# quadjr/aframe-gaussian-splatting

Measured on NVIDIA H100. Metric: frames/sec @1920x1080 (sort + splat raster, 1 M synthetic train-like splats), higher is better.
Workload: dtype f64 sort keys + f32 shading

## Files before the change

### aframe-gaussian-splatting_b200/csrc/gs_project.cu

```cuda
#include "gs_common.cuh"

namespace gs {

__device__ __forceinline__ void unpack_int16(uint32_t value, float &lo, float &hi) {
  const int32_t v = (int32_t)value;
  const int32_t v0 = v >> 16;
  int32_t v1 = v & 0xFFFF;
  if (v & 0x8000) v1 |= (int32_t)0xFFFF0000;
  lo = (float)v1;
  hi = (float)v0;
}

#define MUL(a, b) __fmul_rn((a), (b))
#define ADD(a, b) __fadd_rn((a), (b))
#define SUB(a, b) __fsub_rn((a), (b))
#define DIV(a, b) __fdiv_rn((a), (b))
#define DOT3(a0, b0, a1, b1, a2, b2) ADD(ADD(MUL(a0, b0), MUL(a1, b1)), MUL(a2, b2))

__device__ __forceinline__ uint32_t project_one(const RenderConsts &rc, const float *mv, const float4 c,
                                                const uint4 *__restrict__ cc, uint32_t i, uint32_t j,
                                                float4 *__restrict__ rec_out, uint4 &q, bool &have_q) {
  uint32_t rect = kNoRect;
  const float *P = rc.proj;
  float cam[4], p[4];
// ... 134 lines not shown
    constexpr uint32_t kChunk = 1024;
    __shared__ uint32_t s_list[kChunk];
    __shared__ uint32_t s_warp[8];
    const uint32_t tid = threadIdx.x, lane = tid & 31u, warp = tid >> 5;
    const uint32_t nchunks = (n + kChunk - 1) / kChunk;
    for (uint32_t ch = blockIdx.x; ch < nchunks; ch += gridDim.x) {
      const uint32_t base = ch * kChunk + tid * 4u;
      float d[4];
      if (base + 4u <= n) {
        const float4 v = __ldg((const float4 *)(depth + base));
        d[0] = v.x; d[1] = v.y; d[2] = v.z; d[3] = v.w;
        *(uint4 *)(rect_out + base) = make_uint4(kNoRect, kNoRect, kNoRect, kNoRect);
        if (STEREO) *(uint4 *)(rect_out1 + base) = make_uint4(kNoRect, kNoRect, kNoRect, kNoRect);
      } else {
#pragma unroll
        for (uint32_t k = 0; k < 4; ++k) {
          d[k] = (base + k < n) ? __ldg(depth + base + k) : GS_DEPTH_REJECT;
          if (base + k < n) rect_out[base + k] = kNoRect;
          if (STEREO && base + k < n) rect_out1[base + k] = kNoRect;
        }
      }
      bool f[4];
      uint32_t m = 0;
#pragma unroll
      for (uint32_t k = 0; k < 4; ++k) {
        f[k] = (base + k < n) && ((d[k] != GS_DEPTH_REJECT) || q5_head(base + k));
        m += f[k] ? 1u : 0u;
      }
      uint32_t incl = m;
      for (int o = 1; o < 32; o <<= 1) {
        const uint32_t t = __shfl_up_sync(0xffffffffu, incl, o);
        if (lane >= (uint32_t)o) incl += t;
      }
      if (lane == 31) s_warp[warp] = incl;
      __syncthreads();
      uint32_t pos = incl - m, total = 0;
#pragma unroll
      for (uint32_t w = 0; w < 8; ++w) {
        const uint32_t t = s_warp[w];
        pos += (w < warp) ? t : 0u;
        total += t;
      }
#pragma unroll
      for (uint32_t k = 0; k < 4; ++k)
        if (f[k]) s_list[pos++] = base + k;
      __syncthreads();
      for (uint32_t q = tid; q < total; q += blockDim.x) {
        const uint32_t i = s_list[q];
        uint32_t rect1 = kNoRect;
        const uint32_t rect = shade(i, i, &rect1);
        if (rect != kNoRect) rect_out[i] = rect;
        if (STEREO && rect1 != kNoRect) rect_out1[i] = rect1;
      }
      __syncthreads();
    }
    return;
  }
  for (uint32_t j = blockIdx.x * blockDim.x + threadIdx.x; j < n; j += stride) {
    const uint32_t i = BY_ENTRY ? __ldg(order + j) : j;
    uint32_t rect = kNoRect, rect1 = kNoRect;
    const bool sorted = BY_ENTRY || (__ldg(depth + i) != GS_DEPTH_REJECT) || q5_head(i);
    if (sorted) rect = shade(i, j, &rect1);
    rect_out[j] = rect;
    if (STEREO) rect_out1[j] = rect1;
  }
}


__device__ __forceinline__ uint32_t rect_count(uint32_t r, uint32_t rank, uint32_t world) {
  if (r == kNoRect) return 0u;
  const uint32_t h = (r >> 24) - ((r >> 16) & 255u) + 1u;
  uint32_t w = ((r >> 8) & 255u) - (r & 255u) + 1u;
  if (world > 1) {
    uint32_t first;
    owned_span(r & 255u, (r >> 8) & 255u, rank, world, first, w);
  }
  return w * h;
}

template <bool SLAB, bool STEREO = false>
__global__ void __launch_bounds__(kEmitThreads) k_count(const uint32_t *__restrict__ order,
                                                        const uint32_t *__restrict__ rect,
                                                        uint2 *__restrict__ ent, uint32_t *__restrict__ ent_off,
                                                        uint32_t *__restrict__ slice_total,
                                                        uint32_t *__restrict__ slice_prefix, FrameCounters *ctr,
                                                        const FrameParams *__restrict__ fp,
                                                        const uint32_t *__restrict__ bin_open,
                                                        uint32_t *__restrict__ rect1) {
  GS_PDL_ENTRY();
  const uint32_t shard_rank = fp->rc.shard_rank, shard_world = fp->rc.shard_world;
  __shared__ uint32_t s_warp[kEmitThreads / 32], s_vis[kEmitThreads / 32];
  __shared__ uint32_t s_last;
  const uint32_t tid = threadIdx.x, lane = tid & 31, warp = tid >> 5;
  const uint32_t nv = ctr->sort.n_valid;
  const uint32_t num_slices = (nv + kEmitTile - 1) / kEmitTile;
  for (uint32_t sl = blockIdx.x; sl < num_slices; sl += gridDim.x) {
    const uint32_t j = sl * kEmitTile + tid;
    uint32_t idx = 0, r = kNoRect, r1 = kNoRect;
    if (j < nv) {
      idx = SLAB ? j : __ldg(order + j);
      r = __ldg(rect + idx);
      if (STEREO) r1 = SLAB ? rect1[idx] : __ldg(rect1 + idx);
    }
    auto all_closed = [&](uint32_t rr, uint32_t bin_base) -> bool {
      const uint32_t bx0 = rr & 255u, bx1 = (rr >> 8) & 255u, by0 = (rr >> 16) & 255u, by1 = rr >> 24;
      if ((bx1 - bx0 + 1u) * (by1 - by0 + 1u) > 4u) return false;
      bool any = false;
      for (uint32_t by = by0; by <= by1; ++by)
        for (uint32_t bx = bx0; bx <= bx1; ++bx) any = any || (__ldg(bin_open + bin_base + by * fp->rc.bins_x + bx) != 0u);
      return !any;
    };
    uint32_t cnt = rect_count(r, shard_rank, shard_world);
    if (SLAB && cnt && all_closed(r, 0u)) cnt = 0;
    const uint32_t cnt0 = cnt;
    if (STEREO) {
      uint32_t cnt1 = rect_count(r1, 0u, 1u);
      if (SLAB && cnt1 && all_closed(r1, fp->rc.n_bins)) {
        cnt1 = 0;
        rect1[idx] = kNoRect;
      }
      cnt += cnt1;
    }
    uint32_t incl = cnt, vis = (r != kNoRect) + (STEREO && r1 != kNoRect);
    for (int o = 1; o < 32; o <<= 1) {
      const uint32_t t = __shfl_up_sync(0xffffffffu, incl, o);
      if (lane >= (uint32_t)o) incl += t;
    }
    for (int o = 16; o > 0; o >>= 1) vis += __shfl_xor_sync(0xffffffffu, vis, o);
    if (lane == 31) s_warp[warp] = incl;
    if (lane == 0) s_vis[warp] = vis;
    __syncthreads();
    uint32_t wbase = 0, total = 0, v = 0;
    for (uint32_t k = 0; k < kEmitThreads / 32; ++k) {
      if (k < warp) wbase += s_warp[k];
      total += s_warp[k];
      v += s_vis[k];
    }
    if (j < nv) {
      ent[j] = make_uint2(idx, (SLAB && STEREO ? cnt0 : cnt) ? r : kNoRect);
      ent_off[j] = wbase + incl - cnt;
    }
    if (tid == 0) {
      slice_total[sl] = total;
      if (v) atomicAdd(&ctr->n_visible, v);
    }
    __syncthreads();
  }
  __threadfence();
  __syncthreads();
  if (tid == 0) s_last = (atomicAdd(&ctr->count_done, 1u) == gridDim.x - 1) ? 1u : 0u;
  __syncthreads();
  if (!s_last) return;
  __threadfence();
  unsigned long long carry = 0;
  for (uint32_t b = 0; b < num_slices; b += kEmitThreads) {
    const uint32_t i = b + tid;
    const uint32_t v = (i < num_slices) ? __ldcg(slice_total + i) : 0u;
    uint32_t incl = v;
    for (int o = 1; o < 32; o <<= 1) {
      const uint32_t t = __shfl_up_sync(0xffffffffu, incl, o);
      if (lane >= (uint32_t)o) incl += t;
    }
    __syncthreads();
    if (lane == 31) s_warp[warp] = incl;
    __syncthreads();
    uint32_t wbase = 0, total = 0;
    for (uint32_t k = 0; k < kEmitThreads / 32; ++k) {
      if (k < warp) wbase += s_warp[k];
      total += s_warp[k];
    }
    if (i < num_slices) slice_prefix[i] = (uint32_t)(carry + wbase + incl - v);
    carry += total;
  }
  if (tid == 0) {
    slice_prefix[num_slices] = (uint32_t)(carry > 0xFFFFFFFFull ? 0xFFFFFFFFull : carry);
    ctr->n_inst = carry;
  }
}

__device__ __forceinline__ void emit_candidate(const RenderConsts &rc, uint32_t bx, uint32_t by, bool multi, const float4 &r0,
                                               const float2 &r1, const uint32_t *__restrict__ bin_open, uint32_t payload,
                                               size_t pos, uint16_t *__restrict__ inst_tile, uint32_t *__restrict__ inst_idx,
                                               uint32_t bin_base) {
  bool keep = true;
  if (multi)
    keep = footprint_meets_box(r0.x, r0.y, r0.z, r0.w, r1.x, r1.y, (float)(bx * kBin) + 0.5f, (float)(by * kBin) + 0.5f,
                               (float)(kBin - 1));
  const uint32_t t = bin_base + by * rc.bins_x + bx;
  if (keep && bin_open) keep = __ldg(bin_open + t) != 0u;
  inst_tile[pos] = keep ? (uint16_t)t : kNoTile;
  inst_idx[pos] = payload;
}

template <bool STEREO = false>
__global__ void __launch_bounds__(256) k_emit_entries(const uint2 *__restrict__ ent, const uint32_t *__restrict__ ent_off,
                                                      const uint32_t *__restrict__ slice_prefix,
                                                      const float4 *__restrict__ proj_rec, const FrameParams *__restrict__ fp,
                                                      uint64_t cap_inst, uint16_t *__restrict__ inst_tile,
                                                      uint32_t *__restrict__ inst_idx, FrameCounters *ctr,
                                                      const uint32_t *__restrict__ bin_open,
                                                      const float4 *__restrict__ proj_rec1, const uint32_t *__restrict__ rect1) {
  GS_PDL_ENTRY();
  const RenderConsts &rc = fp->rc;
  const uint32_t nv = ctr->sort.n_valid;
  if (ctr->n_inst > cap_inst) {
    if (blockIdx.x == 0 && threadIdx.x == 0) ctr->overflow = 1u;
    return;
  }
  const uint32_t lane = threadIdx.x & 31u;
  const uint32_t stride = gridDim.x * blockDim.x;
  const uint32_t nv_pad = (nv + 31u) & ~31u;
  for (uint32_t j = blockIdx.x * blockDim.x + threadIdx.x; j < nv_pad; j += stride) {
    uint2 en = make_uint2(0u, kNoRect);
    if (j < nv) en = __ldg(ent + j);
    uint32_t off = 0;
#pragma unroll
    for (uint32_t eye = 0; eye < (STEREO ? 2u : 1u); ++eye) {
      const uint32_t r = eye == 0u ? en.y : (j < nv ? __ldg(rect1 + en.x) : kNoRect);
      const float4 *rec = eye == 0u ? proj_rec : proj_rec1;
      const uint32_t bin_base = eye * rc.n_bins;
      uint32_t bx0 = 0, by0 = 0, w = 0, h = 0, step = 1, n_own = 0;
      size_t base = 0;
      float4 r0 = make_float4(0.f, 0.f, 0.f, 0.f);
      float2 r1 = make_float2(0.f, 0.f);
      bool multi = false;
      if (r != kNoRect) {
        bx0 = r & 255u;
        by0 = (r >> 16) & 255u;
        h = (r >> 24) - by0 + 1u;
        w = ((r >> 8) & 255u) - bx0 + 1u;
        multi = w * h > 1u;
        if (rc.shard_world > 1) {
          owned_span(bx0, (r >> 8) & 255u, rc.shard_rank, rc.shard_world, bx0, w);
          step = rc.shard_world;
        }
        n_own = w * h;
        base = (size_t)__ldg(slice_prefix + (j >> 8)) + __ldg(ent_off + j) + off;
        if (multi) {
          r0 = __ldg(rec + 2 * (size_t)en.x);
          r1 = __ldg((const float2 *)(rec + 2 * (size_t)en.x + 1));
        }
      }
      off += n_own;
      const bool big = n_own > 8u;
      if (!big) {
        for (uint32_t k = 0; k < n_own; ++k) {
          const uint32_t row = k / w;
          emit_candidate(rc, bx0 + (k - row * w) * step, by0 + row, multi, r0, r1, bin_open, en.x, base + k, inst_tile, inst_idx,
                         bin_base);
        }
      }
      uint32_t todo = __ballot_sync(0xffffffffu, big);
      while (todo) {
        const int src = __ffs(todo) - 1;
        todo &= todo - 1;
        const uint32_t s_bx0 = __shfl_sync(0xffffffffu, bx0, src), s_by0 = __shfl_sync(0xffffffffu, by0, src);
        const uint32_t s_w = __shfl_sync(0xffffffffu, w, src), s_step = __shfl_sync(0xffffffffu, step, src);
        const uint32_t s_n = __shfl_sync(0xffffffffu, n_own, src), s_pay = __shfl_sync(0xffffffffu, en.x, src);
        const unsigned long long s_base = __shfl_sync(0xffffffffu, (unsigned long long)base, src);
        float4 g0;
        float2 g1;
        g0.x = __shfl_sync(0xffffffffu, r0.x, src); g0.y = __shfl_sync(0xffffffffu, r0.y, src);
        g0.z = __shfl_sync(0xffffffffu, r0.z, src); g0.w = __shfl_sync(0xffffffffu, r0.w, src);
        g1.x = __shfl_sync(0xffffffffu, r1.x, src); g1.y = __shfl_sync(0xffffffffu, r1.y, src);
        for (uint32_t k = lane; k < s_n; k += 32u) {
          const uint32_t row = k / s_w;
          emit_candidate(rc, s_bx0 + (k - row * s_w) * s_step, s_by0 + row, true, g0, g1, bin_open, s_pay, (size_t)s_base + k,
                         inst_tile, inst_idx, bin_base);
        }
      }
    }
  }
}

void launch_project(gs_context *c, const FrameParams *fp, const FrameCounters *ctr, const FrameBufs &b, cudaStream_t stream) {
  uint64_t blocks = ((uint64_t)c->cap + 255) / 256;
  const uint64_t cap = (uint64_t)c->sm_count * 16;
  if (blocks > cap) blocks = cap;
  if (blocks < 1) blocks = 1;
  launch_chain(c, k_project<false>, (int)blocks, 256, stream, (const float4 *)c->center_scale, (const uint4 *)c->cov_color, (const float *)c->depth, fp, b.proj_rec, b.rect,
               (const uint32_t *)nullptr, ctr, (const SceneTable *)nullptr,
               (const StereoParams *)nullptr, (float4 *)nullptr, (uint32_t *)nullptr);
}

void launch_project_stereo(gs_context *c, const StereoParams *stereo, const SceneTable *scene, const FrameCounters *ctr,
                           const FrameBufs &b, cudaStream_t stream) {
  uint64_t blocks = ((uint64_t)c->cap + 255) / 256;
  const uint64_t cap = (uint64_t)c->sm_count * 16;
  if (blocks > cap) blocks = cap;
  if (blocks < 1) blocks = 1;
  launch_chain(c, k_project<false, true, true>, (int)blocks, 256, stream, (const float4 *)c->center_scale, (const uint4 *)c->cov_color,
               (const float *)c->depth, &stereo->eye[0], b.proj_rec, b.rect, (const uint32_t *)nullptr, ctr, scene, stereo,
               b.proj_rec1, b.rect1);
}

void launch_project_scene(gs_context *c, const FrameParams *fp, const SceneTable *scene, const FrameCounters *ctr,
                          const FrameBufs &b, cudaStream_t stream) {
  uint64_t blocks = ((uint64_t)c->cap + 255) / 256;
  const uint64_t cap = (uint64_t)c->sm_count * 16;
  if (blocks > cap) blocks = cap;
  if (blocks < 1) blocks = 1;
  launch_chain(c, k_project<false, true>, (int)blocks, 256, stream, (const float4 *)c->center_scale, (const uint4 *)c->cov_color,
               (const float *)c->depth, fp, b.proj_rec, b.rect, (const uint32_t *)nullptr, ctr, scene, (const StereoParams *)nullptr,
               (float4 *)nullptr, (uint32_t *)nullptr);
}

void launch_project_entries(gs_context *c, const FrameParams *fp, FrameCounters *ctr, const SceneTable *scene,
                            const StereoParams *stereo, const FrameBufs &b, cudaStream_t stream) {
  uint64_t blocks = ((uint64_t)c->cap + 255) / 256;
  const uint64_t cap = (uint64_t)c->sm_count * 16;
  if (blocks > cap) blocks = cap;
  if (blocks < 1) blocks = 1;
  if (stereo) {
    launch_chain(c, k_project<true, true, true>, (int)blocks, 256, stream, (const float4 *)c->center_scale,
                 (const uint4 *)c->cov_color, (const float *)c->depth, &stereo->eye[0], b.proj_rec, b.rect,
                 (const uint32_t *)b.order, (const FrameCounters *)ctr, scene, stereo, b.proj_rec1, b.rect1);
    return;
  }
  launch_chain(c, scene ? k_project<true, true> : k_project<true>, (int)blocks, 256, stream, (const float4 *)c->center_scale,
               (const uint4 *)c->cov_color, (const float *)c->depth, fp, b.proj_rec, b.rect, (const uint32_t *)b.order,
               (const FrameCounters *)ctr, scene, (const StereoParams *)nullptr, (float4 *)nullptr, (uint32_t *)nullptr);
}

void launch_emit(gs_context *c, const FrameParams *fp, FrameCounters *ctr, const FrameBufs &b, const uint32_t *bin_open,
                 cudaStream_t st) {
  uint64_t tiles = ((uint64_t)c->cap + kEmitTile - 1) / kEmitTile;
  const uint64_t cap = (uint64_t)c->sm_count * 8;
  if (tiles > cap) tiles = cap;
  if (tiles < 1) tiles = 1;
  const bool stereo = b.rect1 != nullptr;
  auto count = bin_open ? (stereo ? k_count<true, true> : k_count<true>) : (stereo ? k_count<false, true> : k_count<false>);
  launch_chain(c, count, (int)tiles, kEmitThreads, st, (const uint32_t *)b.order, (const uint32_t *)b.rect, c->ent, c->ent_off,
               c->slice_total, c->slice_prefix, ctr, fp, bin_open, b.rect1);
  launch_chain(c, stereo ? k_emit_entries<true> : k_emit_entries<false>, (int)tiles, 256, st, (const uint2 *)c->ent, (const uint32_t *)c->ent_off,
               (const uint32_t *)c->slice_prefix, (const float4 *)b.proj_rec, fp, (uint64_t)c->cap_inst, c->inst_tile, c->inst_idx, ctr,
               bin_open, (const float4 *)b.proj_rec1, (const uint32_t *)b.rect1);
}

}
```

### aframe-gaussian-splatting_b200/csrc/gs_sort.cu

```cuda
#include <type_traits>

#include "gs_common.cuh"
#include "gs_depthkey.cuh"

namespace gs {

__device__ __forceinline__ bool worker_keep(const SortConsts &sc, const float4 c, const float s, double &depth) {
  const double x = c.x, y = c.y, z = c.z;
  depth = __dadd_rn(__dadd_rn(__dadd_rn(__dmul_rn(sc.view[0], x), __dmul_rn(sc.view[1], y)), __dmul_rn(sc.view[2], z)),
                    sc.view[3]);
  bool in_box = true;
  if (sc.has_cutout) {
    const double *e = sc.cutout;
    const double ny = -y;
    const double w = __ddiv_rn(
        1.0, __dadd_rn(__dadd_rn(__dadd_rn(__dmul_rn(e[3], x), __dmul_rn(e[7], ny)), __dmul_rn(e[11], z)), e[15]));
    const double c0 = __dmul_rn(
        __dadd_rn(__dadd_rn(__dadd_rn(__dmul_rn(e[0], x), __dmul_rn(e[4], ny)), __dmul_rn(e[8], z)), e[12]), w);
    const double c1 = __dmul_rn(
        __dadd_rn(__dadd_rn(__dadd_rn(__dmul_rn(e[1], x), __dmul_rn(e[5], ny)), __dmul_rn(e[9], z)), e[13]), w);
    const double c2 = __dmul_rn(
        __dadd_rn(__dadd_rn(__dadd_rn(__dmul_rn(e[2], x), __dmul_rn(e[6], ny)), __dmul_rn(e[10], z)), e[14]), w);
    if (c0 < -0.5 || c0 > 0.5 || c1 < -0.5 || c1 > 0.5 || c2 < -0.5 || c2 > 0.5) in_box = false;
  }
// ... 59 lines not shown
      atomicAdd(&ctr->sort.n_valid, cnt);
    }
  }
}

__global__ void __launch_bounds__(256) k_depth_cull_scene(const float4 *__restrict__ cs, const float *__restrict__ sa,
                                                          const FrameParams *__restrict__ fp, const SceneTable *__restrict__ scene,
                                                          float *__restrict__ depth_out, FrameCounters *ctr, ObjCounters *octr) {
  GS_PDL_ENTRY();
  __shared__ uint32_t s_first[kMaxObjects], s_end[kMaxObjects], s_cnt[kMaxObjects];
  __shared__ unsigned long long s_min[kMaxObjects], s_max[kMaxObjects];
  const uint32_t n_obj = scene->n;
  for (uint32_t k = threadIdx.x; k < n_obj; k += blockDim.x) {
    s_first[k] = scene->obj[k].first;
    s_end[k] = scene->obj[k].end;
    s_cnt[k] = 0;
    s_min[k] = 0;
    s_max[k] = 0;
  }
  __syncthreads();
  const uint32_t n = fp->n_splats;
  const uint32_t stride = gridDim.x * blockDim.x;
  int cur = -1;
  double dmin = INFINITY, dmax = -INFINITY;
  uint32_t cnt = 0;
  auto flush = [&]() {
    if (cnt) {
      atomicMax(&s_min[cur], ~enc_f64(dmin));
      atomicMax(&s_max[cur], enc_f64(dmax));
      atomicAdd(&s_cnt[cur], cnt);
    }
    dmin = INFINITY;
    dmax = -INFINITY;
    cnt = 0;
  };
  auto process = [&](uint32_t i, const float4 c, const float s) {
    float out = GS_DEPTH_REJECT;
    const int k = scene_find(s_first, s_end, n_obj, i);
    double depth;
    if (k >= 0 && worker_keep(scene->obj[k].sc, c, s, depth)) {
      if (k != cur) {
        flush();
        cur = k;
      }
      out = (float)depth;
      ++cnt;
      if (depth > dmax) dmax = depth;
      if (depth < dmin) dmin = depth;
    }
    depth_out[i] = out;
  };
  for (uint32_t i = blockIdx.x * blockDim.x + threadIdx.x; i < n; i += 2 * stride) {
    const uint32_t j = i + stride;
    const bool two = j < n;
    const float4 c0 = __ldg(cs + i);
    const float s0 = __ldg(sa + i);
    float4 c1 = c0;
    float s1 = s0;
    if (two) {
      c1 = __ldg(cs + j);
      s1 = __ldg(sa + j);
    }
    process(i, c0, s0);
    if (two) process(j, c1, s1);
  }
  flush();
  __syncthreads();
  for (uint32_t k = threadIdx.x; k < n_obj; k += blockDim.x) {
    if (!s_cnt[k]) continue;
    atomicMax(&octr[k].min_enc, s_min[k]);
    atomicMax(&octr[k].max_enc, s_max[k]);
    atomicAdd(&octr[k].n_valid, s_cnt[k]);
    atomicMax(&ctr->sort.min_enc, s_min[k]);
    atomicMax(&ctr->sort.max_enc, s_max[k]);
    atomicAdd(&ctr->sort.n_valid, s_cnt[k]);
  }
}

__global__ void __launch_bounds__(256) k_scene_keys(const float *__restrict__ depth, const FrameParams *__restrict__ fp,
                                                    const SceneTable *__restrict__ scene, const ObjCounters *__restrict__ octr,
                                                    FrameCounters *ctr, uint32_t *__restrict__ key_out,
                                                    uint32_t *__restrict__ pay_out) {
  GS_PDL_ENTRY();
  __shared__ SceneKeyTable s_ent;
  __shared__ uint32_t s_in, s_drop;
  s_ent.load(scene, octr);
  if (threadIdx.x == 0) { s_in = 0; s_drop = 0; }
  __syncthreads();
  const uint32_t n = ctr->sort.n_valid ? fp->n_splats : 0u;
  uint32_t in = 0, drop = 0;
  for (uint32_t i = blockIdx.x * blockDim.x + threadIdx.x; i < n; i += gridDim.x * blockDim.x) {
    const float d = __ldg(depth + i);
    uint32_t key = kNoKey;
    if (d != GS_DEPTH_REJECT) {
      int k;
      key = s_ent.key(i, d, k);
      if (key & 65536u) {
        pay_out[i] = s_ent.first[k];
        ++drop;
      } else {
        pay_out[i] = i;
        ++in;
      }
    }
    key_out[i] = key;
  }
  for (int o = 16; o > 0; o >>= 1) {
    in += __shfl_xor_sync(0xffffffffu, in, o);
    drop += __shfl_xor_sync(0xffffffffu, drop, o);
  }
  if ((threadIdx.x & 31u) == 0) {
    if (in) atomicAdd(&s_in, in);
    if (drop) atomicAdd(&s_drop, drop);
  }
  __syncthreads();
  if (threadIdx.x == 0) {
    if (s_in) atomicAdd(&ctr->sort.n_inrange, s_in);
    if (s_drop) atomicAdd(&ctr->sort.n_dropped, s_drop);
  }
}

static int persistent_grid(gs_context *c, uint64_t n_elems, int per_cta, int ctas_per_sm) {
  uint64_t tiles = (n_elems + per_cta - 1) / per_cta;
  uint64_t cap = (uint64_t)c->sm_count * ctas_per_sm;
  if (tiles < 1) tiles = 1;
  return (int)(tiles < cap ? tiles : cap);
}

void launch_depth_cull(gs_context *c, const FrameParams *fp, FrameCounters *ctr, cudaStream_t st) {
  const int grid = persistent_grid(c, c->cap, 256 * 4, 8);
  launch_chain(c, k_depth_cull, grid, 256, st, c->center_scale, c->size_alpha, fp, c->depth, ctr);
}

void launch_depth_cull_scene(gs_context *c, const FrameParams *fp, const SceneTable *scene, ObjCounters *octr, FrameCounters *ctr,
                             cudaStream_t st) {
  const int grid = persistent_grid(c, c->cap, 256 * 4, 8);
  launch_chain(c, k_depth_cull_scene, grid, 256, st, c->center_scale, c->size_alpha, fp, scene, c->depth, ctr, octr);
}

void launch_scene_keys(gs_context *c, const FrameParams *fp, const SceneTable *scene, const ObjCounters *octr, FrameCounters *ctr,
                       cudaStream_t st) {
  const int grid = persistent_grid(c, c->cap, 256 * 4, 8);
  launch_chain(c, k_scene_keys, grid, 256, st, (const float *)c->depth, fp, scene, octr, ctr, c->scene_key, c->scene_pay);
}

struct RadixScratch {
  uint32_t *table;
  uint32_t *totals;
  uint32_t stride;
};

struct RadixPass {
  using Carry = void;
  __device__ void prepare(uint32_t n) {}
  __device__ void hist_prologue(uint32_t n) const {}
  __device__ void hist_epilogue() {}
  __device__ void scanned(uint32_t total) const {}
  __device__ void digit_range(uint32_t d, uint32_t start, uint32_t end) const {}
};

template <class Pass>
__global__ void __launch_bounds__(kRadixThreads) k_radix_hist(Pass p, const RadixScratch s) {
  GS_PDL_ENTRY();
  __shared__ uint32_t h[256];
  const uint32_t tid = threadIdx.x, lane = tid & 31, warp = tid >> 5;
  const uint32_t n = p.count();
  const uint32_t num_chunks = (n + kRadixTile - 1) / kRadixTile;
  p.prepare(n);
  p.hist_prologue(n);
  for (uint32_t c = blockIdx.x; c < num_chunks; c += gridDim.x) {
    h[tid] = 0;
    __syncthreads();
    const uint32_t base = c * kRadixTile + warp * (32 * kRadixItems) + lane;
#pragma unroll
    for (int k = 0; k < kRadixItems; ++k) {
      const uint32_t i = base + k * 32;
      if (i < n) {
        uint32_t pay, carry;
        const uint32_t digit = p.load(i, pay, carry);
        if (digit != kInvalidDigit) atomicAdd(&h[digit], 1u);
      }
    }
    __syncthreads();
    s.table[(size_t)tid * s.stride + c] = h[tid];
    __syncthreads();
  }
  p.hist_epilogue();
}

template <class Pass>
__global__ void __launch_bounds__(256) k_radix_scan(const Pass p, const RadixScratch s) {
  GS_PDL_ENTRY();
  __shared__ uint32_t s_warp[8];
  __shared__ uint32_t s_carry;
  const uint32_t tid = threadIdx.x, lane = tid & 31, warp = tid >> 5;
  const uint32_t n = p.count();
  const uint32_t num_chunks = (n + kRadixTile - 1) / kRadixTile;
  uint32_t *row = s.table + (size_t)blockIdx.x * s.stride;
  if (tid == 0) s_carry = 0;
  __syncthreads();
  for (uint32_t b = 0; b < num_chunks; b += 256) {
    const uint32_t i = b + tid;
    const uint32_t v = (i < num_chunks) ? row[i] : 0u;
    uint32_t incl = v;
    for (int o = 1; o < 32; o <<= 1) {
      const uint32_t t = __shfl_up_sync(0xffffffffu, incl, o);
      if (lane >= (uint32_t)o) incl += t;
    }
    if (lane == 31) s_warp[warp] = incl;
    __syncthreads();
    uint32_t wbase = 0;
    for (uint32_t k = 0; k < warp; ++k) wbase += s_warp[k];
    const uint32_t carry = s_carry;
    if (i < num_chunks) row[i] = carry + wbase + incl - v;
    __syncthreads();
    if (tid == 255) s_carry = carry + wbase + incl;
    __syncthreads();
  }
  if (tid == 0) {
    s.totals[blockIdx.x] = s_carry;
    p.scanned(s_carry);
  }
}

constexpr int kScatThreads = 512;
constexpr int kScatItems = kRadixTile / kScatThreads;
constexpr int kScatWarps = kScatThreads / 32;

template <class Pass>
__global__ void __launch_bounds__(kScatThreads, 2) k_radix_scatter(Pass p, const RadixScratch s) {
  GS_PDL_ENTRY();
  constexpr bool kCarry = !std::is_void<typename Pass::Carry>::value;
  using carry_t = typename std::conditional<kCarry, typename Pass::Carry, uint8_t>::type;
  __shared__ uint32_t wcnt[kScatWarps][256];
  __shared__ uint32_t tile_off[256];
  __shared__ uint32_t s_loc[256];
  __shared__ uint32_t s_warp_tot[8];
  __shared__ uint32_t s_pay[kRadixTile];
  __shared__ carry_t s_carry[kCarry ? kRadixTile : 1];
  __shared__ uint8_t s_dig[kRadixTile];
  __shared__ uint32_t s_total;
  const uint32_t tid = threadIdx.x, lane = tid & 31, warp = tid >> 5;
  const uint32_t n = p.count();
  const uint32_t num_chunks = (n + kRadixTile - 1) / kRadixTile;
  if (blockIdx.x >= num_chunks) return;

  auto scan256 = [&](uint32_t v) -> uint32_t {
    uint32_t incl = v;
    for (int o = 1; o < 32; o <<= 1) {
      const uint32_t t = __shfl_up_sync(0xffffffffu, incl, o);
      if (lane >= (uint32_t)o) incl += t;
    }
    __syncthreads();
    if (lane == 31 && warp < 8) s_warp_tot[warp] = incl;
    __syncthreads();
    uint32_t wbase = 0;
    for (uint32_t k = 0; k < warp && k < 8; ++k) wbase += s_warp_tot[k];
    return wbase + incl - v;
  };

  const uint32_t dtot = tid < 256 ? s.totals[tid] : 0u;
  const uint32_t dbase = scan256(dtot);
  if (blockIdx.x == 0 && tid < 256) p.digit_range(tid, dbase, dbase + dtot);
  p.prepare(n);

  for (uint32_t c = blockIdx.x; c < num_chunks; c += gridDim.x) {
    const uint32_t toff = tid < 256 ? __ldg(s.table + (size_t)tid * s.stride + c) : 0u;
    for (uint32_t k = tid; k < kScatWarps * 256; k += kScatThreads) (&wcnt[0][0])[k] = 0u;
    const uint32_t base = c * kRadixTile + warp * (32 * kScatItems) + lane;
    uint32_t digit[kScatItems], pay[kScatItems], rank[kScatItems];
    carry_t carry[kScatItems];
#pragma unroll
    for (int k = 0; k < kScatItems; ++k) {
      const uint32_t i = base + k * 32;
      uint32_t cv = 0;
      digit[k] = kInvalidDigit;
      pay[k] = 0;
      if (i < n) digit[k] = p.load(i, pay[k], cv);
      carry[k] = (carry_t)cv;
    }
    __syncthreads();
#pragma unroll
    for (int k = 0; k < kScatItems; ++k) {
      const uint32_t d = digit[k];
      const uint32_t peers = __match_any_sync(0xffffffffu, d);
      const uint32_t lt = __popc(peers & ((1u << lane) - 1u));
      uint32_t prior = 0;
      if (d != kInvalidDigit) prior = wcnt[warp][d];
      __syncwarp();
      if (d != kInvalidDigit && lt == 0) wcnt[warp][d] = prior + __popc(peers);
      __syncwarp();
      rank[k] = prior + lt;
    }
    __syncthreads();
    uint32_t total = 0;
    if (tid < 256) {
#pragma unroll
      for (int w = 0; w < kScatWarps; ++w) {
        const uint32_t cnt = wcnt[w][tid];
        wcnt[w][tid] = total;
        total += cnt;
      }
    }
    const uint32_t loc = scan256(total);
    if (tid < 256) {
      s_loc[tid] = loc;
      tile_off[tid] = dbase + toff - loc;
      if (tid == 255) s_total = loc + total;
    }
    __syncthreads();
#pragma unroll
    for (int k = 0; k < kScatItems; ++k) {
      const uint32_t d = digit[k];
      if (d == kInvalidDigit) continue;
      const uint32_t lp = s_loc[d] + wcnt[warp][d] + rank[k];
      s_pay[lp] = pay[k];
      s_dig[lp] = (uint8_t)d;
      if (kCarry) s_carry[lp] = carry[k];
    }
    __syncthreads();
    const uint32_t nvalid = s_total;
    for (uint32_t i = tid; i < nvalid; i += kScatThreads)
      p.store(tile_off[s_dig[i]] + i, s_pay[i], kCarry ? (uint32_t)s_carry[i] : 0u);
    __syncthreads();
  }
}

template <class Pass>
static void run_pass(gs_context *c, const Pass &p, const RadixScratch &s, uint64_t n_max, cudaStream_t st) {
  const int grid = persistent_grid(c, n_max, kRadixTile, 8);
  launch_chain(c, k_radix_hist<Pass>, grid, kRadixThreads, st, p, s);
  launch_chain(c, k_radix_scan<Pass>, 256, 256, st, p, s);
  launch_chain(c, k_radix_scatter<Pass>, grid, kScatThreads, st, p, s);
}

struct D1 : RadixPass {
  using Carry = uint8_t;
  FrameCounters *ctr;
  const FrameParams *fp;
  const float *depth;
  uint32_t *idx_out; uint8_t *hi_out;
  DepthRange dr;
  uint32_t n_in, n_drop;
  __device__ uint32_t count() const { return ctr->sort.n_valid ? fp->n_splats : 0u; }
  __device__ void prepare(uint32_t n) { if (n) dr = load_depth_range(ctr); }
  __device__ uint32_t load(uint32_t i, uint32_t &pay, uint32_t &carry) {
    const float d = __ldg(depth + i);
    if (d == GS_DEPTH_REJECT) return kInvalidDigit;
    const int32_t key = depth_key(d, dr.min_depth, dr.depth_inv);
    if (key < 0 || key > 65535) { ++n_drop; return kInvalidDigit; }
    ++n_in;
    pay = i;
    carry = (uint32_t)key >> 8;
    return key & 255;
  }
  __device__ void store(uint32_t pos, uint32_t pay, uint32_t carry) const { idx_out[pos] = pay; hi_out[pos] = (uint8_t)carry; }
  __device__ void hist_epilogue() {
    __shared__ uint32_t s_in, s_drop;
    uint32_t in = n_in, drop = n_drop;
    for (int o = 16; o > 0; o >>= 1) {
      in += __shfl_xor_sync(0xffffffffu, in, o);
      drop += __shfl_xor_sync(0xffffffffu, drop, o);
    }
    if (threadIdx.x == 0) { s_in = 0; s_drop = 0; }
    __syncthreads();
    if ((threadIdx.x & 31u) == 0) { if (in) atomicAdd(&s_in, in); if (drop) atomicAdd(&s_drop, drop); }
    __syncthreads();
    if (threadIdx.x == 0) {
      if (s_in) atomicAdd(&ctr->sort.n_inrange, s_in);
      if (s_drop) atomicAdd(&ctr->sort.n_dropped, s_drop);
    }
  }
};

struct D2 : RadixPass {
  const FrameCounters *ctr;
  const uint8_t *dig; const uint32_t *idx;
  uint32_t *order;
  __device__ uint32_t count() const { return ctr->sort.n_inrange; }
  __device__ void hist_prologue(uint32_t n) const {
    const uint32_t nv = ctr->sort.n_valid;
    for (uint32_t j = n + blockIdx.x * blockDim.x + threadIdx.x; j < nv; j += gridDim.x * blockDim.x) order[j] = 0u;
  }
  __device__ uint32_t load(uint32_t i, uint32_t &pay, uint32_t &) const { pay = idx[i]; return dig[i]; }
  __device__ void store(uint32_t pos, uint32_t pay, uint32_t) const { order[pos] = pay; }
};

void launch_depth_radix(gs_context *c, const FrameParams *fp, FrameCounters *ctr, const FrameBufs &b, cudaStream_t st) {
  const RadixScratch s{c->table_n, c->totals, c->table_n_stride};
  run_pass(c, D1{{}, ctr, fp, c->depth, c->idx_a, c->dig_a}, s, c->cap, st);
  run_pass(c, D2{{}, ctr, c->dig_a, c->idx_a, b.order}, s, c->cap, st);
}

struct M1 : RadixPass {
  using Carry = uint16_t;
  const FrameCounters *ctr;
  const FrameParams *fp;
  const uint32_t *key, *pay_in;
  uint32_t *idx_out; uint16_t *hi_out;
  __device__ uint32_t count() const { return ctr->sort.n_valid ? fp->n_splats : 0u; }
  __device__ uint32_t load(uint32_t i, uint32_t &pay, uint32_t &carry) const {
    const uint32_t k = key[i];
    if (k == kNoKey) return kInvalidDigit;
    carry = k >> 8;
    pay = pay_in[i];
    return k & 255u;
  }
  __device__ void store(uint32_t pos, uint32_t pay, uint32_t carry) const { idx_out[pos] = pay; hi_out[pos] = (uint16_t)carry; }
};

struct M2 : RadixPass {
  using Carry = uint8_t;
  const FrameCounters *ctr;
  const uint16_t *hi; const uint32_t *idx;
  uint32_t *idx_out; uint8_t *hi_out;
  __device__ uint32_t count() const { return ctr->sort.n_valid; }
  __device__ uint32_t load(uint32_t i, uint32_t &pay, uint32_t &carry) const {
    const uint32_t h = hi[i];
    carry = h >> 8;
    pay = idx[i];
    return h & 255u;
  }
  __device__ void store(uint32_t pos, uint32_t pay, uint32_t carry) const { idx_out[pos] = pay; hi_out[pos] = (uint8_t)carry; }
};

struct M3 : RadixPass {
  const FrameCounters *ctr;
  const uint8_t *dig; const uint32_t *idx;
  uint32_t *order;
  __device__ uint32_t count() const { return ctr->sort.n_valid; }
  __device__ uint32_t load(uint32_t i, uint32_t &pay, uint32_t &) const { pay = idx[i]; return dig[i]; }
  __device__ void store(uint32_t pos, uint32_t pay, uint32_t) const { order[pos] = pay; }
};

void launch_scene_radix(gs_context *c, const FrameParams *fp, FrameCounters *ctr, const FrameBufs &b, cudaStream_t st) {
  const RadixScratch s{c->table_n, c->totals, c->table_n_stride};
  run_pass(c, M1{{}, ctr, fp, c->scene_key, c->scene_pay, c->idx_a, c->scene_hi}, s, c->cap, st);
  run_pass(c, M2{{}, ctr, c->scene_hi, c->idx_a, c->scene_pay, c->dig_a}, s, c->cap, st);
  run_pass(c, M3{{}, ctr, c->dig_a, c->scene_pay, b.order}, s, c->cap, st);
}

struct S1 : RadixPass {
  using Carry = uint8_t;
  const FrameCounters *ctr;
  const uint16_t *key; const uint32_t *idx;
  uint32_t *idx_out; uint8_t *hi_out;
  __device__ uint32_t count() const { return ctr->sort.n_valid; }
  __device__ uint32_t load(uint32_t i, uint32_t &pay, uint32_t &carry) const {
    const uint32_t k = key[i];
    carry = k >> 8;
    pay = idx[i];
    return k & 255u;
  }
  __device__ void store(uint32_t pos, uint32_t pay, uint32_t carry) const { idx_out[pos] = pay; hi_out[pos] = (uint8_t)carry; }
};

struct SM1 : RadixPass {
  using Carry = uint16_t;
  const FrameCounters *ctr;
  const SceneTable *scene;
  const uint32_t *key, *idx;
  uint32_t *idx_out; uint16_t *hi_out;
  __device__ uint32_t count() const { return ctr->sort.n_valid; }
  __device__ uint32_t load(uint32_t i, uint32_t &pay, uint32_t &carry) const {
    const uint32_t k = key[i];
    carry = k >> 8;
    pay = idx[i];
    if (k & 65536u) {
      uint32_t lo = 0, hi = scene->n;
      while (hi - lo > 1) {
        const uint32_t mid = (lo + hi) >> 1;
        if (scene->obj[mid].first <= pay) lo = mid; else hi = mid;
      }
      pay = scene->obj[lo].first;
    }
    return k & 255u;
  }
  __device__ void store(uint32_t pos, uint32_t pay, uint32_t carry) const { idx_out[pos] = pay; hi_out[pos] = (uint16_t)carry; }
};

void launch_slab_sort(gs_context *c, const FrameParams *fp, FrameCounters *ctr, const SceneTable *scene, const FrameBufs &b,
                      cudaStream_t st) {
  const RadixScratch s{c->table_n, c->totals, c->table_n_stride};
  if (scene) {
    run_pass(c, SM1{{}, ctr, scene, c->scene_key, c->cidx, c->idx_a, c->scene_hi}, s, c->cap, st);
    run_pass(c, M2{{}, ctr, c->scene_hi, c->idx_a, c->scene_pay, c->dig_a}, s, c->cap, st);
    run_pass(c, M3{{}, ctr, c->dig_a, c->scene_pay, b.order}, s, c->cap, st);
    return;
  }
  run_pass(c, S1{{}, ctr, c->ckey, c->cidx, c->idx_a, c->dig_a}, s, c->cap, st);
  run_pass(c, D2{{}, ctr, c->dig_a, c->idx_a, b.order}, s, c->cap, st);
}

__device__ __forceinline__ void gather_record(const float4 *rec, float4 *inst_rec, uint32_t splat, uint32_t pos) {
  const float4 r0 = __ldg(rec + 2 * (size_t)splat);
  const float4 r1 = __ldg(rec + 2 * (size_t)splat + 1);
  inst_rec[2 * (size_t)pos] = r0;
  inst_rec[2 * (size_t)pos + 1] = r1;
}

struct T1 : RadixPass {
  using Carry = uint16_t;
  FrameCounters *ctr;
  const uint16_t *bin; const uint32_t *idx;
  uint16_t *bin_out; uint32_t *idx_out;
  const float4 *proj_rec; float4 *inst_rec; uint2 *bin_range;
  uint32_t n_bins;
  bool last;
  __device__ uint32_t count() const { return ctr->overflow ? 0u : (uint32_t)ctr->n_inst; }
  __device__ uint32_t load(uint32_t i, uint32_t &pay, uint32_t &carry) const {
    const uint16_t t = bin[i];
    if (t == kNoTile) return kInvalidDigit;
    carry = t;
    pay = idx[i];
    return t & 255;
  }
  __device__ void store(uint32_t pos, uint32_t pay, uint32_t carry) const {
    if (last) gather_record(proj_rec, inst_rec, pay, pos);
    else { idx_out[pos] = pay; bin_out[pos] = (uint16_t)carry; }
  }
  __device__ void scanned(uint32_t total) const { if (total) atomicAdd(&ctr->n_inst_kept, total); }
  __device__ void digit_range(uint32_t d, uint32_t start, uint32_t end) const {
    if (last && d < n_bins) bin_range[d] = make_uint2(start, end);
  }
};

struct T2 : RadixPass {
  using Carry = uint16_t;
  const FrameCounters *ctr;
  const uint16_t *bin; const uint32_t *idx;
  const float4 *proj_rec; float4 *inst_rec; uint16_t *bin_out;
  __device__ uint32_t count() const { return ctr->overflow ? 0u : ctr->n_inst_kept; }
  __device__ uint32_t load(uint32_t i, uint32_t &pay, uint32_t &carry) const {
    const uint16_t t = bin[i];
    carry = t;
    pay = idx[i];
    return (uint32_t)t >> 8;
  }
  __device__ void store(uint32_t pos, uint32_t pay, uint32_t carry) const {
    gather_record(proj_rec, inst_rec, pay, pos);
    bin_out[pos] = (uint16_t)carry;
  }
};

__global__ void __launch_bounds__(256) k_tile_ranges(const uint16_t *__restrict__ tile_f, FrameCounters *ctr,
                                                     uint2 *__restrict__ range) {
  GS_PDL_ENTRY();
  const uint32_t n = ctr->overflow ? 0u : ctr->n_inst_kept;
  for (uint32_t i = blockIdx.x * blockDim.x + threadIdx.x; i < n; i += gridDim.x * blockDim.x) {
    const uint32_t t = tile_f[i];
    if (i == 0 || tile_f[i - 1] != t) range[t].x = i;
    if (i == n - 1 || tile_f[i + 1] != t) range[t].y = i + 1;
  }
}

struct T1S : T1 {
  const float4 *proj_rec1;
  uint32_t eye_bins;
  __device__ void store(uint32_t pos, uint32_t pay, uint32_t carry) const {
    if (last) gather_record(carry >= eye_bins ? proj_rec1 : proj_rec, inst_rec, pay, pos);
    else { idx_out[pos] = pay; bin_out[pos] = (uint16_t)carry; }
  }
};
struct T2S : T2 {
  const float4 *proj_rec1;
  uint32_t eye_bins;
  __device__ void store(uint32_t pos, uint32_t pay, uint32_t carry) const {
    gather_record(carry >= eye_bins ? proj_rec1 : proj_rec, inst_rec, pay, pos);
    bin_out[pos] = (uint16_t)carry;
  }
};

void launch_tile_radix(gs_context *c, FrameCounters *ctr, const FrameBufs &b, uint32_t n_bins, cudaStream_t st) {
  const RadixScratch s{c->table_d, c->totals + 256, c->table_d_stride};
  const bool last = n_bins <= 256u;
  if (b.proj_rec1) {
    const T1 t1{{}, ctr, c->inst_tile, c->inst_idx, c->inst_tile_b, c->inst_idx_b, b.proj_rec, b.inst_rec, b.bin_range, n_bins, last};
    run_pass(c, T1S{t1, b.proj_rec1, n_bins / 2}, s, c->cap_inst, st);
    if (last) return;
    const T2 t2{{}, ctr, c->inst_tile_b, c->inst_idx_b, b.proj_rec, b.inst_rec, c->inst_tile_f};
    run_pass(c, T2S{t2, b.proj_rec1, n_bins / 2}, s, c->cap_inst, st);
    launch_chain(c, k_tile_ranges, persistent_grid(c, c->cap_inst, 256 * 8, 8), 256, st, (const uint16_t *)c->inst_tile_f, ctr,
                 b.bin_range);
    return;
  }
  run_pass(c, T1{{}, ctr, c->inst_tile, c->inst_idx, c->inst_tile_b, c->inst_idx_b, b.proj_rec, b.inst_rec, b.bin_range, n_bins, last},
           s, c->cap_inst, st);
  if (last) return;
  run_pass(c, T2{{}, ctr, c->inst_tile_b, c->inst_idx_b, b.proj_rec, b.inst_rec, c->inst_tile_f}, s, c->cap_inst, st);
  launch_chain(c, k_tile_ranges, persistent_grid(c, c->cap_inst, 256 * 8, 8), 256, st, (const uint16_t *)c->inst_tile_f, ctr,
               b.bin_range);
}

template <int kShift>
struct P : RadixPass {
  const uint32_t *key, *perm;
  uint32_t *perm_out;
  uint32_t n;
  __device__ uint32_t count() const { return n; }
  __device__ uint32_t load(uint32_t i, uint32_t &pay, uint32_t &) const {
    const uint32_t row = kShift == 0 ? i : perm[i];
    pay = row;
    return (__ldg(key + row) >> kShift) & 255u;
  }
  __device__ void store(uint32_t pos, uint32_t pay, uint32_t) const { perm_out[pos] = pay; }
};

uint32_t *launch_ply_sort(gs_context *c, const uint32_t *key, uint32_t *perm_a, uint32_t *perm_b, uint32_t *table,
                          uint32_t *totals, uint32_t n, cudaStream_t st) {
  const RadixScratch s{table, totals, (n + kRadixTile - 1) / kRadixTile + 1};
  run_pass(c, P<0>{{}, key, nullptr, perm_a, n}, s, n, st);
  run_pass(c, P<8>{{}, key, perm_a, perm_b, n}, s, n, st);
  run_pass(c, P<16>{{}, key, perm_b, perm_a, n}, s, n, st);
  run_pass(c, P<24>{{}, key, perm_a, perm_b, n}, s, n, st);
  return perm_b;
}

}
```

Baseline: 3017.

## Batch radix loads, ballot-based peer matching, batched gather, and per-thread slice scan

Splits radix pass loads into fetch/decode so all key loads in a tile are issued before any is used. Replaces __match_any_sync with a ballot-based digit peer mask. Adds a batched record-gather path in the scatter kernel for tile-sort passes. The slice prefix scan now handles 16 elements per thread with 64-bit sums, and the slice prefix load in emit is hoisted out of the eye loop. Together these aim to raise memory-level parallelism and cut latency in the sort and emit stages, at the cost of extra registers and more template plumbing.

Measured after the change: 3033, median of 6. About the same (+0.5%).

```diff
diff --git a/aframe-gaussian-splatting_b200/csrc/gs_project.cu b/aframe-gaussian-splatting_b200/csrc/gs_project.cu
--- a/aframe-gaussian-splatting_b200/csrc/gs_project.cu
+++ b/aframe-gaussian-splatting_b200/csrc/gs_project.cu
@@ -310,24 +310,35 @@
   __syncthreads();
   if (!s_last) return;
   __threadfence();
+  constexpr uint32_t kScanPer = 16;
+  __shared__ unsigned long long s_wsum[kEmitThreads / 32];
   unsigned long long carry = 0;
-  for (uint32_t b = 0; b < num_slices; b += kEmitThreads) {
-    const uint32_t i = b + tid;
-    const uint32_t v = (i < num_slices) ? __ldcg(slice_total + i) : 0u;
-    uint32_t incl = v;
+  for (uint32_t b = 0; b < num_slices; b += kEmitThreads * kScanPer) {
+    const uint32_t first = b + tid * kScanPer;
+    uint32_t v[kScanPer];
+#pragma unroll
+    for (uint32_t k = 0; k < kScanPer; ++k) v[k] = (first + k < num_slices) ? __ldcg(slice_total + first + k) : 0u;
+    unsigned long long sum = 0;
+#pragma unroll
+    for (uint32_t k = 0; k < kScanPer; ++k) sum += v[k];
+    unsigned long long incl = sum;
     for (int o = 1; o < 32; o <<= 1) {
-      const uint32_t t = __shfl_up_sync(0xffffffffu, incl, o);
+      const unsigned long long t = __shfl_up_sync(0xffffffffu, incl, o);
       if (lane >= (uint32_t)o) incl += t;
     }
     __syncthreads();
-    if (lane == 31) s_warp[warp] = incl;
+    if (lane == 31) s_wsum[warp] = incl;
     __syncthreads();
-    uint32_t wbase = 0, total = 0;
+    unsigned long long pos = carry + incl - sum, total = 0;
     for (uint32_t k = 0; k < kEmitThreads / 32; ++k) {
-      if (k < warp) wbase += s_warp[k];
-      total += s_warp[k];
-    }
-    if (i < num_slices) slice_prefix[i] = (uint32_t)(carry + wbase + incl - v);
+      if (k < warp) pos += s_wsum[k];
+      total += s_wsum[k];
+    }
+#pragma unroll
+    for (uint32_t k = 0; k < kScanPer; ++k) {
+      if (first + k < num_slices) slice_prefix[first + k] = (uint32_t)pos;
+      pos += v[k];
+    }
     carry += total;
   }
   if (tid == 0) {
@@ -370,7 +381,11 @@
   const uint32_t nv_pad = (nv + 31u) & ~31u;
   for (uint32_t j = blockIdx.x * blockDim.x + threadIdx.x; j < nv_pad; j += stride) {
     uint2 en = make_uint2(0u, kNoRect);
-    if (j < nv) en = __ldg(ent + j);
+    size_t first = 0;
+    if (j < nv) {
+      en = __ldg(ent + j);
+      first = (size_t)__ldg(slice_prefix + (j >> 8)) + __ldg(ent_off + j);
+    }
     uint32_t off = 0;
 #pragma unroll
     for (uint32_t eye = 0; eye < (STEREO ? 2u : 1u); ++eye) {
@@ -393,7 +408,7 @@
           step = rc.shard_world;
         }
         n_own = w * h;
-        base = (size_t)__ldg(slice_prefix + (j >> 8)) + __ldg(ent_off + j) + off;
+        base = first + off;
         if (multi) {
           r0 = __ldg(rec + 2 * (size_t)en.x);
           r1 = __ldg((const float2 *)(rec + 2 * (size_t)en.x + 1));
diff --git a/aframe-gaussian-splatting_b200/csrc/gs_sort.cu b/aframe-gaussian-splatting_b200/csrc/gs_sort.cu
--- a/aframe-gaussian-splatting_b200/csrc/gs_sort.cu
+++ b/aframe-gaussian-splatting_b200/csrc/gs_sort.cu
@@ -235,6 +235,7 @@
 
 struct RadixPass {
   using Carry = void;
+  static constexpr bool kGather = false;
   __device__ void prepare(uint32_t n) {}
   __device__ void hist_prologue(uint32_t n) const {}
   __device__ void hist_epilogue() {}
@@ -249,21 +250,29 @@
   const uint32_t tid = threadIdx.x, lane = tid & 31, warp = tid >> 5;
   const uint32_t n = p.count();
   const uint32_t num_chunks = (n + kRadixTile - 1) / kRadixTile;
+  using raw_t = typename Pass::Raw;
   p.prepare(n);
   p.hist_prologue(n);
   for (uint32_t c = blockIdx.x; c < num_chunks; c += gridDim.x) {
     h[tid] = 0;
-    __syncthreads();
     const uint32_t base = c * kRadixTile + warp * (32 * kRadixItems) + lane;
+    raw_t raw[kRadixItems];
 #pragma unroll
     for (int k = 0; k < kRadixItems; ++k) {
       const uint32_t i = base + k * 32;
-      if (i < n) {
-        uint32_t pay, carry;
-        const uint32_t digit = p.load(i, pay, carry);
-        if (digit != kInvalidDigit) atomicAdd(&h[digit], 1u);
-      }
-    }
+      raw[k] = i < n ? p.fetch(i) : raw_t();
+    }
+    uint32_t digit[kRadixItems];
+#pragma unroll
+    for (int k = 0; k < kRadixItems; ++k) {
+      const uint32_t i = base + k * 32;
+      uint32_t pay, carry;
+      digit[k] = i < n ? p.decode(i, raw[k], pay, carry) : kInvalidDigit;
+    }
+    __syncthreads();
+#pragma unroll
+    for (int k = 0; k < kRadixItems; ++k)
+      if (digit[k] != kInvalidDigit) atomicAdd(&h[digit[k]], 1u);
     __syncthreads();
     s.table[(size_t)tid * s.stride + c] = h[tid];
     __syncthreads();
@@ -309,12 +318,26 @@
 constexpr int kScatThreads = 512;
 constexpr int kScatItems = kRadixTile / kScatThreads;
 constexpr int kScatWarps = kScatThreads / 32;
+constexpr int kGatherBatch = 2;
+
+__device__ __forceinline__ uint32_t digit_peers(uint32_t d) {
+  const bool valid = d != kInvalidDigit;
+  const uint32_t v = __ballot_sync(0xffffffffu, valid);
+  uint32_t peers = valid ? v : ~v;
+#pragma unroll
+  for (int b = 0; b < 8; ++b) {
+    const uint32_t m = __ballot_sync(0xffffffffu, (d >> b) & 1u);
+    peers &= ((d >> b) & 1u) ? m : ~m;
+  }
+  return peers;
+}
 
 template <class Pass>
 __global__ void __launch_bounds__(kScatThreads, 2) k_radix_scatter(Pass p, const RadixScratch s) {
   GS_PDL_ENTRY();
   constexpr bool kCarry = !std::is_void<typename Pass::Carry>::value;
   using carry_t = typename std::conditional<kCarry, typename Pass::Carry, uint8_t>::type;
+  using raw_t = typename Pass::Raw;
   __shared__ uint32_t wcnt[kScatWarps][256];
   __shared__ uint32_t tile_off[256];
   __shared__ uint32_t s_loc[256];
@@ -353,20 +376,26 @@
     const uint32_t base = c * kRadixTile + warp * (32 * kScatItems) + lane;
     uint32_t digit[kScatItems], pay[kScatItems], rank[kScatItems];
     carry_t carry[kScatItems];
+    raw_t raw[kScatItems];
+#pragma unroll
+    for (int k = 0; k < kScatItems; ++k) {
+      const uint32_t i = base + k * 32;
+      raw[k] = i < n ? p.fetch(i) : raw_t();
+    }
 #pragma unroll
     for (int k = 0; k < kScatItems; ++k) {
       const uint32_t i = base + k * 32;
       uint32_t cv = 0;
       digit[k] = kInvalidDigit;
       pay[k] = 0;
-      if (i < n) digit[k] = p.load(i, pay[k], cv);
+      if (i < n) digit[k] = p.decode(i, raw[k], pay[k], cv);
       carry[k] = (carry_t)cv;
     }
     __syncthreads();
 #pragma unroll
     for (int k = 0; k < kScatItems; ++k) {
       const uint32_t d = digit[k];
-      const uint32_t peers = __match_any_sync(0xffffffffu, d);
+      const uint32_t peers = digit_peers(d);
       const uint32_t lt = __popc(peers & ((1u << lane) - 1u));
       uint32_t prior = 0;
       if (d != kInvalidDigit) prior = wcnt[warp][d];
@@ -403,6 +432,32 @@
     }
     __syncthreads();
     const uint32_t nvalid = s_total;
+    if constexpr (Pass::kGather) {
+      if (p.gathers()) {
+        for (uint32_t b = 0; b < nvalid; b += kGatherBatch * kScatThreads) {
+          const uint32_t i0 = b + tid;
+          float4 r0[kGatherBatch], r1[kGatherBatch];
+          uint32_t pos[kGatherBatch], cr[kGatherBatch];
+#pragma unroll
+          for (int k = 0; k < kGatherBatch; ++k) {
+            const uint32_t i = i0 + k * kScatThreads;
+            if (i < nvalid) {
+              pos[k] = tile_off[s_dig[i]] + i;
+              cr[k] = kCarry ? (uint32_t)s_carry[i] : 0u;
+              const float4 *rec = p.rec_of(cr[k]) + 2 * (size_t)s_pay[i];
+              r0[k] = __ldg(rec);
+              r1[k] = __ldg(rec + 1);
+            }
+          }
+          __syncwarp();
+#pragma unroll
+          for (int k = 0; k < kGatherBatch; ++k)
+            if (i0 + k * kScatThreads < nvalid) p.put(pos[k], cr[k], r0[k], r1[k]);
+        }
+        __syncthreads();
+        continue;
+      }
+    }
     for (uint32_t i = tid; i < nvalid; i += kScatThreads)
       p.store(tile_off[s_dig[i]] + i, s_pay[i], kCarry ? (uint32_t)s_carry[i] : 0u);
     __syncthreads();
@@ -425,10 +480,11 @@
   uint32_t *idx_out; uint8_t *hi_out;
   DepthRange dr;
   uint32_t n_in, n_drop;
+  using Raw = float;
   __device__ uint32_t count() const { return ctr->sort.n_valid ? fp->n_splats : 0u; }
   __device__ void prepare(uint32_t n) { if (n) dr = load_depth_range(ctr); }
-  __device__ uint32_t load(uint32_t i, uint32_t &pay, uint32_t &carry) {
-    const float d = __ldg(depth + i);
+  __device__ float fetch(uint32_t i) const { return __ldg(depth + i); }
+  __device__ uint32_t decode(uint32_t i, float d, uint32_t &pay, uint32_t &carry) {
     if (d == GS_DEPTH_REJECT) return kInvalidDigit;
     const int32_t key = depth_key(d, dr.min_depth, dr.depth_inv);
     if (key < 0 || key > 65535) { ++n_drop; return kInvalidDigit; }
@@ -460,12 +516,14 @@
   const FrameCounters *ctr;
   const uint8_t *dig; const uint32_t *idx;
   uint32_t *order;
+  using Raw = uint8_t;
   __device__ uint32_t count() const { return ctr->sort.n_inrange; }
   __device__ void hist_prologue(uint32_t n) const {
     const uint32_t nv = ctr->sort.n_valid;
     for (uint32_t j = n + blockIdx.x * blockDim.x + threadIdx.x; j < nv; j += gridDim.x * blockDim.x) order[j] = 0u;
   }
-  __device__ uint32_t load(uint32_t i, uint32_t &pay, uint32_t &) const { pay = idx[i]; return dig[i]; }
+  __device__ uint8_t fetch(uint32_t i) const { return dig[i]; }
+  __device__ uint32_t decode(uint32_t i, uint8_t d, uint32_t &pay, uint32_t &) const { pay = idx[i]; return d; }
   __device__ void store(uint32_t pos, uint32_t pay, uint32_t) const { order[pos] = pay; }
 };
 
@@ -481,9 +539,10 @@
   const FrameParams *fp;
   const uint32_t *key, *pay_in;
   uint32_t *idx_out; uint16_t *hi_out;
+  using Raw = uint32_t;
   __device__ uint32_t count() const { return ctr->sort.n_valid ? fp->n_splats : 0u; }
-  __device__ uint32_t load(uint32_t i, uint32_t &pay, uint32_t &carry) const {
-    const uint32_t k = key[i];
+  __device__ uint32_t fetch(uint32_t i) const { return key[i]; }
+  __device__ uint32_t decode(uint32_t i, uint32_t k, uint32_t &pay, uint32_t &carry) const {
     if (k == kNoKey) return kInvalidDigit;
     carry = k >> 8;
     pay = pay_in[i];
@@ -497,9 +556,10 @@
   const FrameCounters *ctr;
   const uint16_t *hi; const uint32_t *idx;
   uint32_t *idx_out; uint8_t *hi_out;
+  using Raw = uint16_t;
   __device__ uint32_t count() const { return ctr->sort.n_valid; }
-  __device__ uint32_t load(uint32_t i, uint32_t &pay, uint32_t &carry) const {
-    const uint32_t h = hi[i];
+  __device__ uint16_t fetch(uint32_t i) const { return hi[i]; }
+  __device__ uint32_t decode(uint32_t i, uint32_t h, uint32_t &pay, uint32_t &carry) const {
     carry = h >> 8;
     pay = idx[i];
     return h & 255u;
@@ -511,8 +571,10 @@
   const FrameCounters *ctr;
   const uint8_t *dig; const uint32_t *idx;
   uint32_t *order;
+  using Raw = uint8_t;
   __device__ uint32_t count() const { return ctr->sort.n_valid; }
-  __device__ uint32_t load(uint32_t i, uint32_t &pay, uint32_t &) const { pay = idx[i]; return dig[i]; }
+  __device__ uint8_t fetch(uint32_t i) const { return dig[i]; }
+  __device__ uint32_t decode(uint32_t i, uint8_t d, uint32_t &pay, uint32_t &) const { pay = idx[i]; return d; }
   __device__ void store(uint32_t pos, uint32_t pay, uint32_t) const { order[pos] = pay; }
 };
 
@@ -528,9 +590,10 @@
   const FrameCounters *ctr;
   const uint16_t *key; const uint32_t *idx;
   uint32_t *idx_out; uint8_t *hi_out;
+  using Raw = uint16_t;
   __device__ uint32_t count() const { return ctr->sort.n_valid; }
-  __device__ uint32_t load(uint32_t i, uint32_t &pay, uint32_t &carry) const {
-    const uint32_t k = key[i];
+  __device__ uint16_t fetch(uint32_t i) const { return key[i]; }
+  __device__ uint32_t decode(uint32_t i, uint32_t k, uint32_t &pay, uint32_t &carry) const {
     carry = k >> 8;
     pay = idx[i];
     return k & 255u;
@@ -544,9 +607,10 @@
   const SceneTable *scene;
   const uint32_t *key, *idx;
   uint32_t *idx_out; uint16_t *hi_out;
+  using Raw = uint32_t;
   __device__ uint32_t count() const { return ctr->sort.n_valid; }
-  __device__ uint32_t load(uint32_t i, uint32_t &pay, uint32_t &carry) const {
-    const uint32_t k = key[i];
+  __device__ uint32_t fetch(uint32_t i) const { return key[i]; }
+  __device__ uint32_t decode(uint32_t i, uint32_t k, uint32_t &pay, uint32_t &carry) const {
     carry = k >> 8;
     pay = idx[i];
     if (k & 65536u) {
@@ -575,13 +639,6 @@
   run_pass(c, D2{{}, ctr, c->dig_a, c->idx_a, b.order}, s, c->cap, st);
 }
 
-__device__ __forceinline__ void gather_record(const float4 *rec, float4 *inst_rec, uint32_t splat, uint32_t pos) {
-  const float4 r0 = __ldg(rec + 2 * (size_t)splat);
-  const float4 r1 = __ldg(rec + 2 * (size_t)splat + 1);
-  inst_rec[2 * (size_t)pos] = r0;
-  inst_rec[2 * (size_t)pos + 1] = r1;
-}
-
 struct T1 : RadixPass {
   using Carry = uint16_t;
   FrameCounters *ctr;
@@ -590,17 +647,22 @@
   const float4 *proj_rec; float4 *inst_rec; uint2 *bin_range;
   uint32_t n_bins;
   bool last;
+  using Raw = uint16_t;
   __device__ uint32_t count() const { return ctr->overflow ? 0u : (uint32_t)ctr->n_inst; }
-  __device__ uint32_t load(uint32_t i, uint32_t &pay, uint32_t &carry) const {
-    const uint16_t t = bin[i];
+  __device__ uint16_t fetch(uint32_t i) const { return bin[i]; }
+  __device__ uint32_t decode(uint32_t i, uint16_t t, uint32_t &pay, uint32_t &carry) const {
+    pay = idx[i];
     if (t == kNoTile) return kInvalidDigit;
     carry = t;
-    pay = idx[i];
     return t & 255;
   }
-  __device__ void store(uint32_t pos, uint32_t pay, uint32_t carry) const {
-    if (last) gather_record(proj_rec, inst_rec, pay, pos);
-    else { idx_out[pos] = pay; bin_out[pos] = (uint16_t)carry; }
+  __device__ void store(uint32_t pos, uint32_t pay, uint32_t carry) const { idx_out[pos] = pay; bin_out[pos] = (uint16_t)carry; }
+  static constexpr bool kGather = true;
+  __device__ bool gathers() const { return last; }
+  __device__ const float4 *rec_of(uint32_t) const { return proj_rec; }
+  __device__ void put(uint32_t pos, uint32_t, float4 r0, float4 r1) const {
+    inst_rec[2 * (size_t)pos] = r0;
+    inst_rec[2 * (size_t)pos + 1] = r1;
   }
   __device__ void scanned(uint32_t total) const { if (total) atomicAdd(&ctr->n_inst_kept, total); }
   __device__ void digit_range(uint32_t d, uint32_t start, uint32_t end) const {
@@ -613,15 +675,21 @@
   const FrameCounters *ctr;
   const uint16_t *bin; const uint32_t *idx;
   const float4 *proj_rec; float4 *inst_rec; uint16_t *bin_out;
+  using Raw = uint16_t;
   __device__ uint32_t count() const { return ctr->overflow ? 0u : ctr->n_inst_kept; }
-  __device__ uint32_t load(uint32_t i, uint32_t &pay, uint32_t &carry) const {
-    const uint16_t t = bin[i];
+  __device__ uint16_t fetch(uint32_t i) const { return bin[i]; }
+  __device__ uint32_t decode(uint32_t i, uint16_t t, uint32_t &pay, uint32_t &carry) const {
     carry = t;
     pay = idx[i];
     return (uint32_t)t >> 8;
   }
-  __device__ void store(uint32_t pos, uint32_t pay, uint32_t carry) const {
-    gather_record(proj_rec, inst_rec, pay, pos);
+  __device__ void store(uint32_t, uint32_t, uint32_t) const {}
+  static constexpr bool kGather = true;
+  __device__ bool gathers() const { return true; }
+  __device__ const float4 *rec_of(uint32_t) const { return proj_rec; }
+  __device__ void put(uint32_t pos, uint32_t carry, float4 r0, float4 r1) const {
+    inst_rec[2 * (size_t)pos] = r0;
+    inst_rec[2 * (size_t)pos + 1] = r1;
     bin_out[pos] = (uint16_t)carry;
   }
 };
@@ -640,18 +708,12 @@
 struct T1S : T1 {
   const float4 *proj_rec1;
   uint32_t eye_bins;
-  __device__ void store(uint32_t pos, uint32_t pay, uint32_t carry) const {
-    if (last) gather_record(carry >= eye_bins ? proj_rec1 : proj_rec, inst_rec, pay, pos);
-    else { idx_out[pos] = pay; bin_out[pos] = (uint16_t)carry; }
-  }
+  __device__ const float4 *rec_of(uint32_t carry) const { return carry >= eye_bins ? proj_rec1 : proj_rec; }
 };
 struct T2S : T2 {
   const float4 *proj_rec1;
   uint32_t eye_bins;
-  __device__ void store(uint32_t pos, uint32_t pay, uint32_t carry) const {
-    gather_record(carry >= eye_bins ? proj_rec1 : proj_rec, inst_rec, pay, pos);
-    bin_out[pos] = (uint16_t)carry;
-  }
+  __device__ const float4 *rec_of(uint32_t carry) const { return carry >= eye_bins ? proj_rec1 : proj_rec; }
 };
 
 void launch_tile_radix(gs_context *c, FrameCounters *ctr, const FrameBufs &b, uint32_t n_bins, cudaStream_t st) {
@@ -680,11 +742,12 @@
   const uint32_t *key, *perm;
   uint32_t *perm_out;
   uint32_t n;
+  using Raw = uint32_t;
   __device__ uint32_t count() const { return n; }
-  __device__ uint32_t load(uint32_t i, uint32_t &pay, uint32_t &) const {
-    const uint32_t row = kShift == 0 ? i : perm[i];
-    pay = row;
-    return (__ldg(key + row) >> kShift) & 255u;
+  __device__ uint32_t fetch(uint32_t i) const { return kShift == 0 ? __ldg(key + i) : perm[i]; }
+  __device__ uint32_t decode(uint32_t i, uint32_t r, uint32_t &pay, uint32_t &) const {
+    pay = kShift == 0 ? i : r;
+    return ((kShift == 0 ? r : __ldg(key + r)) >> kShift) & 255u;
   }
   __device__ void store(uint32_t pos, uint32_t pay, uint32_t) const { perm_out[pos] = pay; }
 };
```
